# rdesc/autorally

Hardware: AMD Instinct MI355X
Metric: trajectory rollouts/s per MPPI solve (higher is better)
Workload: dtype f32

## Files before the change

### autorally_amd/csrc/group_roles.hpp

```cpp
#pragma once

#include "mppi_device.hpp"
#include "noise_device.hpp"

namespace mppi {

constexpr int kGRing = 16;
constexpr int kGCtlChunk = 4;

template <class SH>
struct GroupRoles {
  static constexpr int kPose = SH::NW, kCost = SH::NW + 1, kCtl = SH::NW + 2, kRng = SH::NW + 3;
  static constexpr int kWaves = SH::NW + 4;
  static_assert(kWaves <= (int)(sizeof(SH::fin) / sizeof(int)), "fin[]");
  static_assert(SH::kR == 16 || SH::kR == 8, "rollouts per group");
};
template <class SH>
__device__ __forceinline__ int group_j(int slot) { return slot & (SH::kR - 1); }
template <class SH>
__device__ __forceinline__ bool group_real(int slot) { return slot < SH::kR; }

template <class SH>
__device__ __forceinline__ int group_seq_min(SH &sh)
{
  int m = lds_peek(lds_addr(&sh.xseq[0][0]));
#pragma unroll
  for (int w = 1; w < SH::NW; w++) m = min(m, lds_peek(lds_addr(&sh.xseq[w][0])));
  return m;
}

struct MrgHalf {
  uint32_t s0, s1, s2;
};
__device__ __forceinline__ uint32_t fold_m(uint64_t x, uint32_t C, uint32_t m)
{
  x = (x >> 32) * C + (x & 0xffffffffULL);
  x = (x >> 32) * C + (x & 0xffffffffULL);
  x = (x >> 32) * C + (x & 0xffffffffULL);
  if (x >= m) x -= m;
  return (uint32_t)x;
}
template <class SH>
__device__ __forceinline__ MrgHalf group_rng_load(const RolloutArgs &a)
{
  const int lane = threadIdx.x & 63;
  const int j = group_j<SH>((lane >> 1) & 15), c = lane & 1;
  const int k = (int)blockIdx.x * SH::kR + j;
  const int K = a.K;
  MrgHalf g{0, 0, 0};
  if (a.inline_noise != 0 && lane < 2 * kRolloutsPerWave) {
    g.s0 = a.rng_in[(3 * c) * K + k]; g.s1 = a.rng_in[(3 * c + 1) * K + k]; g.s2 = a.rng_in[(3 * c + 2) * K + k];
  }
  return g;
}
template <class SH, bool PRE = false>
__device__ __forceinline__ void group_rng_wave(const RolloutArgs &a, SH &sh, const MrgHalf pre = MrgHalf{0, 0, 0})
{
  using R = GroupRoles<SH>;
  const int lane = threadIdx.x & 63;
  const int j = group_j<SH>((lane >> 1) & 15), c = lane & 1;
  const int k = (int)blockIdx.x * SH::kR + j;
  const int K = a.K, T = a.T;
  const bool active = lane < 2 * kRolloutsPerWave;
  const bool real = lane < 2 * SH::kR;
  int budget = spin_budget_init(a.spin_budget, T, a.fault_wave == R::kRng + 1);
  if (a.inline_noise != 0) {
    const uint32_t m = c ? (uint32_t)kM2 : (uint32_t)kM1, C = c ? kC2 : kC1;
    const uint32_t A = c ? (uint32_t)kA21 : (uint32_t)kA12, Bn = c ? (uint32_t)kA23N : (uint32_t)kA13N;
    MrgHalf g{0, 0, 0};
    if constexpr (PRE) {
      g = pre;
    } else if (active) {
      g.s0 = a.rng_in[(3 * c) * K + k]; g.s1 = a.rng_in[(3 * c + 1) * K + k]; g.s2 = a.rng_in[(3 * c + 2) * K + k];
    }
    const uint32_t a_ctl = lds_addr(&sh.ctl_pub[0]);
    const uint32_t a_mypub = lds_addr(&sh.rng_pub[lane]);
    int seen = 0;
    for (int t = 0; t < T; t++) {
      float2 e = make_float2(0.5f, 0.5f);
#ifdef MPPI_DIAG_NORNG
      e = make_float2(0.25f + 0.001f * (float)t, 0.5f);
#else
#pragma unroll
      for (int d = 0; d < 2; d++) {
        const uint32_t p = fold_m((uint64_t)A * (c ? g.s2 : g.s1) + (uint64_t)Bn * (m - g.s0), C, m);
        g.s0 = g.s1; g.s1 = g.s2; g.s2 = p;
        const uint32_t p2 = (uint32_t)__builtin_amdgcn_mov_dpp((int)p, 0xB1, 0xF, 0xF, false);
        uint32_t z = (p >= p2) ? p - p2 : p + (uint32_t)kM1 - p2;
        if (z == 0) z = (uint32_t)kM1;
        const float u = (float)z * 0x1p-32f;
        if (d == 0) e.x = u; else e.y = u;
      }
#endif
      const int need = t - kGRing + 1;
      while (seen < need && --budget > 0) {
        seen = lds_peek(a_ctl);
        if (seen < need) __builtin_amdgcn_s_sleep(2);
      }
      if (active && c == 0) *reinterpret_cast<float2 *>(&sh.eps[t & (kGRing - 1)][j][0]) = e;
      lds_publish(a_mypub, t + 1);
    }
    if (real) {
      a.rng_out[(3 * c) * K + k] = g.s0; a.rng_out[(3 * c + 1) * K + k] = g.s1; a.rng_out[(3 * c + 2) * K + k] = g.s2;
    }
  }
  spin_finish(budget, lds_addr(&sh.fail[0]), lds_addr(&sh.fin[R::kRng]));
}

template <class SH>
__device__ __forceinline__ void group_control_wave(const RolloutArgs &a, SH &sh, const uint32_t a_gate_open = 0)
{
  using R = GroupRoles<SH>;
  constexpr int NSW = SH::NSW;
  static_assert(kGCtlChunk == 4 && kGRing >= 2 * kGCtlChunk, "four steps per iteration, lanes 16 q + j");
  const int lane = threadIdx.x & 63;
  const int j = group_j<SH>(lane & 15), q = lane >> 4;
  const bool real = group_real<SH>(lane & 15);
  const int k = (int)blockIdx.x * SH::kR + j;
  const int K = a.K, T = a.T;
  const bool inl = a.inline_noise != 0;
  float2 *const noise = reinterpret_cast<float2 *>(a.noise);
  const float2 *const Useq = reinterpret_cast<const float2 *>(a.U);
  const bool noise_free_k = (k == 0);
  const bool pure_noise_k = (k >= a.k99);
  const uint32_t a_cd = lds_addr(&sh.cost_done[0]);
  const uint32_t a_mypub = lds_addr(&sh.ctl_pub[lane]);
  const uint32_t a_rng = lds_addr(&sh.rng_pub[0]);
  int budget = spin_budget_init(a.spin_budget, T, a.fault_wave == R::kCtl + 1);
  const bool gated = a_gate_open != 0;
  if (gated)
    while (lds_peek(a_gate_open) == 0 && --budget > 0) __builtin_amdgcn_s_sleep(1);
  int seen_x = 0, seen_c = 0, seen_r = 0;
  for (int t0 = 0, n = 1; t0 < T; t0 += n, n = kGCtlChunk) {
    const int t = t0 + q;
    const bool live = (t < T) & (q < n);
    const int tl = live ? t : T - 1;
    float2 Ut;
    if (gated) {
      const unsigned long long ub = __hip_atomic_load(reinterpret_cast<const unsigned long long *>(Useq + tl), __ATOMIC_RELAXED, __HIP_MEMORY_SCOPE_SYSTEM);
      Ut = make_float2(__uint_as_float((unsigned)ub), __uint_as_float((unsigned)(ub >> 32)));
    } else {
      Ut = Useq[tl];
    }
    float2 e = (live && !inl) ? noise[(size_t)tl * K + k] : make_float2(0.0f, 0.0f);
    const int tm = min(t0 + n, T) - 1;
    const int need_x = (tm >= kGRing) ? (tm - kGRing) * NSW + 1 : 0;
    const int need_c = tm - kGRing + 1;
    while ((seen_x < need_x || seen_c < need_c) && --budget > 0) {
      seen_x = group_seq_min(sh);
      seen_c = lds_peek(a_cd);
      if (seen_x < need_x || seen_c < need_c) __builtin_amdgcn_s_sleep(2);
    }
    if (inl) {
      while (seen_r < tm + 1 && --budget > 0) {
        seen_r = lds_peek(a_rng);
        if (seen_r < tm + 1) __builtin_amdgcn_s_sleep(1);
      }
#ifdef MPPI_DIAG_NOBM
      e = *reinterpret_cast<const float2 *>(&sh.eps[tl & (kGRing - 1)][j][0]);
#else
      e = box_muller(*reinterpret_cast<const float2 *>(&sh.eps[tl & (kGRing - 1)][j][0]));
#endif
    }
    if (live) {
      const bool nf = noise_free_k | (t < a.opt_delay);
      const float n0 = e.x * a.nu[0], n1 = e.y * a.nu[1];
      const float du0 = nf ? 0.0f : n0, du1 = nf ? 0.0f : n1;
      float u0 = nf ? Ut.x : (pure_noise_k ? n0 : Ut.x + n0);
      float u1 = nf ? Ut.y : (pure_noise_k ? n1 : Ut.y + n1);
      if (real) noise[(size_t)t * K + k] = make_float2(u0, u1);
      u0 = clampf(u0, a.u_lo[0], a.u_hi[0]);
      u1 = clampf(u1, a.u_lo[1], a.u_hi[1]);
      const int slot = t & (kGRing - 1);
      sh.ctl_b1[slot][j] = u0;
      sh.ctl_b1[slot][kRolloutsPerWave + j] = u1;
      *reinterpret_cast<float4 *>(&sh.ctl_rec[slot][j][0]) = make_float4(u0, u1, du0, du1);
    }
    lds_publish(a_mypub, tm + 1);
  }
  spin_finish(budget, lds_addr(&sh.fail[0]), lds_addr(&sh.fin[R::kCtl]));
}

template <class SH, bool AFFINE>
__device__ __forceinline__ void group_pose_wave(const RolloutArgs &a, SH &sh)
{
  using R = GroupRoles<SH>;
  constexpr int NSW = SH::NSW;
  static_assert(SH::kR == 16, "one step per iteration: 16-rollout groups only");
  const int lane = threadIdx.x & 63;
  const int j = lane & 15;
  const int T = a.T;
  const uint32_t a_seq0 = lds_addr(&sh.xseq[0][0]);
  const uint32_t a_cd = lds_addr(&sh.cost_done[0]);
  const uint32_t a_mypub = lds_addr(&sh.pose_pub[lane]);
  float x = a.state[0], y = a.state[1], yaw = a.state[2];
  int budget = spin_budget_init(a.spin_budget, T, a.fault_wave == R::kPose + 1), seen = 0, cdone = 0;
  float tf_p = 0.0f, tb_p = 0.0f;
  for (int t = 0; t <= T; t++) {
    float tf = 0.0f, tb = 0.0f;
    if (t < T) {
      const int need = t * NSW + 1;
      while (seen < need && --budget > 0) {
        seen = SH::kRecByAll ? group_seq_min(sh) : lds_peek(a_seq0);
        if (seen < need) __builtin_amdgcn_s_sleep(1);
      }
      const float4 r0 = *reinterpret_cast<const float4 *>(&sh.rec[t & (kGRing - 1)][j][0]);
      float spsi, cpsi;
#ifdef MPPI_DIAG_NOPOSE
      spsi = 0.0f; cpsi = 1.0f; tf = x; tb = y;
#else
      sincos_fast(yaw, spsi, cpsi);
      const float st[3] = {x, y, yaw};
      track_fetch<AFFINE>(a.cost, st, cpsi, spsi, tf, tb);
#endif
      const float sd0 = fmaf(cpsi, r0.y, -(spsi * r0.z));
      const float sd1 = fmaf(spsi, r0.y, cpsi * r0.z);
      const float sd2 = a.negate_yaw_der ? -r0.w : r0.w;
      x = fmaf(sd0, a.dt, x);
      y = fmaf(sd1, a.dt, y);
      yaw = fmaf(sd2, a.dt, yaw);
    }
    if (t > 0) {
      while (cdone < t - kGRing && --budget > 0) cdone = lds_peek(a_cd);
      if (lane < kRolloutsPerWave) *reinterpret_cast<float2 *>(&sh.tex[(t - 1) & (kGRing - 1)][lane][0]) = make_float2(tf_p, tb_p);
      lds_publish(a_mypub, t);
    }
    tf_p = tf; tb_p = tb;
  }
  spin_finish(budget, lds_addr(&sh.fail[0]), lds_addr(&sh.fin[R::kPose]));
}

template <int Q>
__device__ __forceinline__ float quad_bc(float v)
{
  return __int_as_float(__builtin_amdgcn_mov_dpp(__float_as_int(v), Q * 0x55, 0xF, 0xF, false));
}
__device__ __forceinline__ void quad_chain(float v, float d, float dt, int q, float &vq, float &v_out)
{
  const float v1 = fmaf(quad_bc<0>(d), dt, v);
  const float v2 = fmaf(quad_bc<1>(d), dt, v1);
  const float v3 = fmaf(quad_bc<2>(d), dt, v2);
  v_out = fmaf(quad_bc<3>(d), dt, v3);
  const float lo = (q == 0) ? v : v1, hi = (q == 2) ? v2 : v3;
  vq = (q < 2) ? lo : hi;
}
template <class SH, bool AFFINE>
__device__ __forceinline__ void group_pose_wave4(const RolloutArgs &a, SH &sh, const float x0, const float y0, const float yaw0,
                                                 const int budget_cut = 0);
template <class SH, bool AFFINE>
__device__ __forceinline__ void group_pose_wave4(const RolloutArgs &a, SH &sh)
{
  group_pose_wave4<SH, AFFINE>(a, sh, a.state[0], a.state[1], a.state[2]);
}
template <class SH, bool AFFINE>
__device__ __forceinline__ void group_pose_wave4(const RolloutArgs &a, SH &sh, const float x0, const float y0, const float yaw0,
                                                 const int budget_cut)
{
  using R = GroupRoles<SH>;
  constexpr int NSW = SH::NSW;
  static_assert(kRolloutsPerWave == 16 && kGRing >= 8, "lane = 4 j + q");
  const int lane = threadIdx.x & 63;
  const int j = group_j<SH>(lane >> 2), q = lane & 3;
  const int T = a.T;
  const uint32_t a_seq0 = lds_addr(&sh.xseq[0][0]);
  const uint32_t a_cd = lds_addr(&sh.cost_done[0]);
  const uint32_t a_mypub = lds_addr(&sh.pose_pub[lane]);
  float x = x0, y = y0, yaw = yaw0;
  int budget = spin_budget_init(a.spin_budget, T, a.fault_wave == R::kPose + 1 || budget_cut != 0), seen = 0, cdone = 0;
  for (int t0 = 0; t0 < T; t0 += 4) {
    const int t = t0 + q;
    const int tend = min(t0 + 4, T);
    const int need = (tend - 1) * NSW + 1;
    while (seen < need && --budget > 0) {
      seen = SH::kRecByAll ? group_seq_min(sh) : lds_peek(a_seq0);
      if (seen < need) __builtin_amdgcn_s_sleep(1);
    }
    const float4 r0 = *reinterpret_cast<const float4 *>(&sh.rec[t & (kGRing - 1)][j][0]);
    float yaw_q, yaw_n, x_q, x_n, y_q, y_n;
    quad_chain(yaw, a.negate_yaw_der ? -r0.w : r0.w, a.dt, q, yaw_q, yaw_n);
    float spsi, cpsi, tf = 0.0f, tb = 0.0f;
#ifdef MPPI_DIAG_NOPOSE
    spsi = 0.0f; cpsi = 1.0f;
#else
    sincos_fast(yaw_q, spsi, cpsi);
#endif
    quad_chain(x, fmaf(cpsi, r0.y, -(spsi * r0.z)), a.dt, q, x_q, x_n);
    quad_chain(y, fmaf(spsi, r0.y, cpsi * r0.z), a.dt, q, y_q, y_n);
#ifdef MPPI_DIAG_NOPOSE
    tf = x_q; tb = y_q;
#else
    const float st[3] = {x_q, y_q, yaw_q};
    track_fetch<AFFINE>(a.cost, st, cpsi, spsi, tf, tb);
#endif
    x = x_n; y = y_n; yaw = yaw_n;
    while (cdone < tend - kGRing && --budget > 0) cdone = lds_peek(a_cd);
    if (t < T) *reinterpret_cast<float2 *>(&sh.tex[t & (kGRing - 1)][j][0]) = make_float2(tf, tb);
    lds_publish(a_mypub, tend);
  }
  spin_finish(budget, lds_addr(&sh.fail[0]), lds_addr(&sh.fin[R::kPose]));
}

template <class SH>
__device__ __forceinline__ float group_settle(SH &sh, int budget, float J)
{
  using R = GroupRoles<SH>;
  const int lane = threadIdx.x & 63;
  const uint32_t a_fin = lds_addr(&sh.fin[(lane < R::kWaves) ? lane : 0]);
  for (;;) {
    const int v = (lane == R::kCost) ? 1 : lds_peek_lanes(a_fin);
    const bool all = __builtin_amdgcn_ballot_w64(v != 0) == ~0ull;
    if (all || --budget <= 0) break;
    __builtin_amdgcn_s_sleep(1);
  }
  if (budget <= 0 || lds_peek(lds_addr(&sh.fail[0])) != 0) J = __builtin_nanf("");
  return J;
}

template <class SH, bool CTRL>
__device__ __forceinline__ void group_cost_wave(const RolloutArgs &a, SH &sh)
{
  using R = GroupRoles<SH>;
  const int lane = threadIdx.x & 63;
  static_assert(SH::kR == 16, "one step per iteration: 16-rollout groups only");
  const int j = lane & 15;
  const int k = (int)blockIdx.x * kRolloutsPerWave + j;
  const int T = a.T;
  const uint32_t a_mydone = lds_addr(&sh.cost_done[lane]);
  const uint32_t a_pose = lds_addr(&sh.pose_pub[0]);
  int crash = 0, budget = spin_budget_init(a.spin_budget, T, a.fault_wave == R::kCost + 1), seen = 0;
  float J = 0.0f;
  for (int t = 0; t < T; t++) {
    const double rt = a.inv_t[t];
    while (seen < t + 1 && --budget > 0) {
      seen = lds_peek(a_pose);
      if (seen < t + 1) __builtin_amdgcn_s_sleep(1);
    }
    const float4 r0 = *reinterpret_cast<const float4 *>(&sh.rec[t & (kGRing - 1)][j][0]);
    const float4 r1 = *reinterpret_cast<const float4 *>(&sh.ctl_rec[t & (kGRing - 1)][j][0]);
    const float2 tx = *reinterpret_cast<const float2 *>(&sh.tex[t & (kGRing - 1)][j][0]);
    lds_publish(a_mydone, t + 1);
    const int rc = (int)((t > 0) & (fabsf(r0.x) >= kRollCrash));
#ifdef MPPI_DIAG_NOCOST
    crash |= rc;
    int crash_new = crash;
    const float Jn = J + r0.y + r1.x + tx.x + (float)rt;
#else
    CostTerms ct;
    cost_terms_a<CTRL>(a.cost, a.nu, r0.y, r0.z, r1.x, r1.y, r1.z, r1.w, ct);
    crash |= rc;
    int crash_new = crash;
    const float c = cost_terms_b(a.cost, ct, tx.x, tx.y, crash_new);
    const float Jn = running_mean(J, c, t, rt);
#endif
    J = (t > 0) ? Jn : J;
    crash = (t > 0) ? crash_new : crash;
  }
  J = group_settle(sh, budget, J);
  a.costs[k] = J + 0.0f;
}

template <int Q>
__device__ __forceinline__ int quad_bc_i(int v)
{
  return __builtin_amdgcn_mov_dpp(v, Q * 0x55, 0xF, 0xF, false);
}
template <class SH, bool CTRL>
__device__ __forceinline__ void group_cost_wave4(const RolloutArgs &a, SH &sh)
{
  using R = GroupRoles<SH>;
  const int lane = threadIdx.x & 63;
  const int j = group_j<SH>(lane >> 2), q = lane & 3;
  const int k = (int)blockIdx.x * SH::kR + j;
  const int T = a.T;
  const uint32_t a_mydone = lds_addr(&sh.cost_done[lane]);
  const uint32_t a_pose = lds_addr(&sh.pose_pub[0]);
  int crash = 0, budget = spin_budget_init(a.spin_budget, T, a.fault_wave == R::kCost + 1), seen = 0;
  float J = 0.0f;
  for (int t0 = 0; t0 < T; t0 += 4) {
    const int t = t0 + q;
    const int tend = min(t0 + 4, T);
    while (seen < tend && --budget > 0) {
      seen = lds_peek(a_pose);
      if (seen < tend) __builtin_amdgcn_s_sleep(1);
    }
    const float4 r0 = *reinterpret_cast<const float4 *>(&sh.rec[t & (kGRing - 1)][j][0]);
    const float4 r1 = *reinterpret_cast<const float4 *>(&sh.ctl_rec[t & (kGRing - 1)][j][0]);
    const float2 tx = *reinterpret_cast<const float2 *>(&sh.tex[t & (kGRing - 1)][j][0]);
    lds_publish(a_mydone, tend);
    const bool counted = (t > 0) & (t < T);
    int e = (int)(fabsf(r0.x) >= kRollCrash) | (int)(tx.x >= a.cost.boundary_threshold) | (int)(tx.y >= a.cost.boundary_threshold);
    e = counted ? e : 0;
    const int c0 = crash | quad_bc_i<0>(e), c1 = c0 | quad_bc_i<1>(e), c2 = c1 | quad_bc_i<2>(e), c3 = c2 | quad_bc_i<3>(e);
    const int lo = (q == 0) ? c0 : c1, hi = (q == 2) ? c2 : c3;
    int crash_q = (q < 2) ? lo : hi;
    crash = c3;
#ifdef MPPI_DIAG_NOCOST
    const float c = r0.y + r1.x + tx.x + (float)crash_q;
#else
    CostTerms ct;
    cost_terms_a<CTRL>(a.cost, a.nu, r0.y, r0.z, r1.x, r1.y, r1.z, r1.w, ct);
    const float c = cost_terms_b(a.cost, ct, tx.x, tx.y, crash_q);
#endif
#pragma unroll
    for (int l = 0; l < 4; l++) {
      const int tl = t0 + l;
      const float cl = (l == 0) ? quad_bc<0>(c) : (l == 1) ? quad_bc<1>(c) : (l == 2) ? quad_bc<2>(c) : quad_bc<3>(c);
      if (tl > 0 && tl < T) {
#ifdef MPPI_DIAG_NOCOST
        J = J + cl + (float)a.inv_t[tl];
#else
        J = running_mean(J, cl, tl, a.inv_t[tl]);
#endif
      }
    }
  }
  J = group_settle(sh, budget, J);
  if (q == 0 && group_real<SH>(lane >> 2)) a.costs[k] = J + 0.0f;
}

}
```

### autorally_amd/csrc/rollout_row.hip

```cpp
#include "group_roles.hpp"
#include "mppi_kernels.hpp"

namespace mppi {

#ifdef MPPI_ROW_STAMPS
__device__ unsigned long long g_row_stamps[16];
#define RSTAMP(i)                                                                                         \
  do {                                                                                                    \
    if (blockIdx.x == 0 && (threadIdx.x & 63) == 0) {                                                     \
      unsigned long long t__;                                                                             \
      asm volatile("s_memtime %0\n\ts_waitcnt lgkmcnt(0)" : "=s"(t__)::"memory");                           \
      g_row_stamps[i] = t__;                                                                              \
    }                                                                                                     \
  } while (0)
#else
#define RSTAMP(i) do { } while (0)
#endif

template <int H>
struct RowShared {
  static constexpr int NW = 4;
  static constexpr int NSW = 1;
  static constexpr bool kRecByAll = true;
  static constexpr int kR = 16;
  int xseq[NW][64];
  float rec[kGRing][kRolloutsPerWave][4];
  int cost_done[64];
  float ctl_b1[kGRing][64];
  float ctl_rec[kGRing][kRolloutsPerWave][4];
  int ctl_pub[64];
  float tex[kGRing][kRolloutsPerWave][2];
  int pose_pub[64];
  float eps[kGRing][kRolloutsPerWave][2];
  int rng_pub[64];
  int fail[4];
  int fin[8];
  float gstate[8];
  int gate_open[8];
  float dump[NW][64 * 2 + (kGRing - 1) * kRolloutsPerWave * 4];
};

template <int H, bool TREE>
struct RowWeights {
  f32x2 w1[kNetIn], w2[H], w3[TREE ? 4 : H];
  f32x2 b1s, b2s, b3;
};

constexpr int kRowPackEntries = 40;
template <int H, bool TREE>
__device__ __forceinline__ void row_load(const float *rowpack, int p, RowWeights<H, TREE> &W)
{
  static_assert(H == 32, "entry layout of pack_row_weights");
  const float4 *pk = reinterpret_cast<const float4 *>(rowpack) + p;
#pragma unroll
  for (int i = 0; i < 3; i++) {
    const float4 v = pk[i * 16];
    W.w1[2 * i] = f32x2{v.x, v.y};
    W.w1[2 * i + 1] = f32x2{v.z, v.w};
  }
#pragma unroll
  for (int i = 0; i < H / 2; i++) {
    const float4 v = pk[(3 + i) * 16];
    W.w2[2 * i] = f32x2{v.x, v.y};
    W.w2[2 * i + 1] = f32x2{v.z, v.w};
    if constexpr (!TREE) {
      const float4 u = pk[(3 + H / 2 + i) * 16];
      W.w3[2 * i] = f32x2{u.x, u.y};
      W.w3[2 * i + 1] = f32x2{u.z, u.w};
    }
  }
  const float4 b = pk[35 * 16];
  W.b1s = f32x2{b.x, b.y};
  W.b2s = f32x2{b.z, b.w};
  if constexpr (TREE) {
    const float4 u = pk[37 * 16], v = pk[38 * 16], c = pk[39 * 16];
    W.w3[0] = f32x2{u.x, u.y};
    W.w3[1] = f32x2{u.z, u.w};
    W.w3[2] = f32x2{v.x, v.y};
    W.w3[3] = f32x2{v.z, v.w};
    W.b3 = f32x2{c.x, c.y};
  } else {
    const float4 c = pk[36 * 16];
    W.b3 = f32x2{c.x, c.y};
  }
}

template <int Q>
__device__ __forceinline__ float row_bc(float a)
{
  return __int_as_float(__builtin_amdgcn_mov_dpp(__float_as_int(a), 0x150 + Q, 0xF, 0xF, false));
}
template <int Q>
__device__ __forceinline__ f32x2 row_bc2(f32x2 a)
{
  return __builtin_bit_cast(f32x2, (long long)__builtin_amdgcn_mov_dpp(__builtin_bit_cast(long long, a), 0x150 + Q, 0xF, 0xF, false));
}
template <int Q>
__device__ __forceinline__ void row_dot_step(f32x2 &z, f32x2 &b, const f32x2 *w, f32x2 a)
{
  z = __builtin_elementwise_fma(w[2 * Q], f32x2{b.x, b.x}, z);
  __builtin_amdgcn_sched_barrier(0);
  const f32x2 bn = row_bc2<(Q + 1 < 16 ? Q + 1 : 15)>(a);
  __builtin_amdgcn_sched_barrier(0);
  z = __builtin_elementwise_fma(w[2 * Q + 1], f32x2{b.y, b.y}, z);
  __builtin_amdgcn_sched_barrier(0);
  b = bn;
}
__device__ __forceinline__ f32x2 row_dot_bc(const f32x2 *w, f32x2 a)
{
  f32x2 z = {0.0f, 0.0f};
  f32x2 b = row_bc2<0>(a);
  __builtin_amdgcn_sched_barrier(0);
#define RD4(Q) row_dot_step<Q>(z, b, w, a); row_dot_step<Q + 1>(z, b, w, a); row_dot_step<Q + 2>(z, b, w, a); row_dot_step<Q + 3>(z, b, w, a);
  RD4(0) RD4(4) RD4(8) RD4(12)
#undef RD4
  return z;
}

template <int CTRL>
__device__ __forceinline__ float dpp_add(float acc, float src)
{
  return acc + __int_as_float(__builtin_amdgcn_update_dpp(0, __float_as_int(src), CTRL, 0xF, 0xF, true));
}
__device__ __forceinline__ float row_out_tree(const f32x2 *w3, f32x2 a)
{
  const f32x2 ax = {a.x, a.x}, ay = {a.y, a.y};
  const f32x2 v01 = __builtin_elementwise_fma(w3[1], ay, w3[0] * ax);
  const f32x2 v23 = __builtin_elementwise_fma(w3[3], ay, w3[2] * ax);
  float v0 = dpp_add<0x128>(v01.x, v23.x);
  const float v1 = dpp_add<0x128>(v01.y, v23.y);
  v0 = dpp_add<0x141>(v0, v1);
  v0 = dpp_add<0xB1>(v0, v0);
  v0 = dpp_add<0x4E>(v0, v0);
  return v0;
}

template <int H, bool TREE, bool GATED = false>
__device__ __forceinline__ void row_dynamics(const RolloutArgs &a, RowShared<H> &sh, const int w)
{
  static_assert(H == 32, "row_dot_bc: 32 activations, two per lane of a 16-lane row");
  const int lane = threadIdx.x & 63;
  const int r = lane >> 4, p = lane & 15;
  const int jr = 4 * w + r;
  const bool odd = (p & 1) != 0;
  const int T = a.T;
  RowWeights<H, TREE> W;
  row_load<H, TREE>(a.wpack, p, W);
#pragma unroll
  for (int k = 0; k < H; k++) asm volatile("" : "+v"(W.w2[k]));
#pragma unroll
  for (int k = 0; k < (TREE ? 4 : H); k++) asm volatile("" : "+v"(W.w3[k]));

  const uint32_t a_myseq = lds_addr(&sh.xseq[w][lane]);
  typedef const volatile int __attribute__((address_space(3))) *lds_int_p;
  typedef const volatile f32x2 __attribute__((address_space(3))) *lds_f2_p;
  const lds_int_p p_pub = (lds_int_p)&sh.ctl_pub[0];
  const lds_f2_p p_u = (lds_f2_p)&sh.ctl_rec[0][jr][0];
  constexpr int kSlotF2 = kRolloutsPerWave * 2;
  const uint32_t a_rec0 = TREE ? (((p & 3) == 0) ? lds_addr(&sh.rec[0][jr][p >> 2]) : lds_addr(&sh.dump[w][2 * lane]))
                               : ((p < 2) ? lds_addr(&sh.rec[0][jr][2 * p]) : lds_addr(&sh.dump[w][2 * lane]));
  constexpr uint32_t kRecStride = sizeof(float) * kRolloutsPerWave * 4;

  int budget = spin_budget_init(a.spin_budget, T, a.fault_wave == w + 1);
  f32x2 sp;
  if constexpr (GATED) {
    const uint32_t a_go = lds_addr(&sh.gate_open[0]);
    while (lds_peek(a_go) == 0 && --budget > 0) __builtin_amdgcn_s_sleep(1);
    const volatile float *gs = sh.gstate;
    sp = TREE ? f32x2{gs[3 + (p >> 2)], 0.0f} : odd ? f32x2{gs[5], gs[6]} : f32x2{gs[3], gs[4]};
  } else {
    sp = TREE ? f32x2{a.state[3 + (p >> 2)], 0.0f} : odd ? f32x2{a.state[5], a.state[6]} : f32x2{a.state[3], a.state[4]};
  }
  if (w == 0) RSTAMP(2);
  while (__builtin_amdgcn_readfirstlane(*p_pub) < 1 && --budget > 0) __builtin_amdgcn_s_sleep(1);
  if (w == 0) RSTAMP(3);
  f32x2 un = p_u[0];
  asm volatile("" : "+v"(un));

  for (int t = 0; t < T - 1; t++) {
    const int slot = t & (kGRing - 1);
    const f32x2 u = un;
    const f32x2 slo = TREE ? f32x2{row_bc<0>(sp.x), row_bc<4>(sp.x)} : f32x2{row_bc<0>(sp.x), row_bc<0>(sp.y)};
    const f32x2 shi = TREE ? f32x2{row_bc<8>(sp.x), row_bc<12>(sp.x)} : f32x2{row_bc<1>(sp.x), row_bc<1>(sp.y)};
    if constexpr (TREE) asm volatile("ds_write_b32 %0, %1" ::"v"(a_rec0 + (uint32_t)slot * kRecStride), "v"(sp.x) : "memory");
    else asm volatile("ds_write_b64 %0, %1" ::"v"(a_rec0 + (uint32_t)slot * kRecStride), "v"(sp) : "memory");
    lds_publish(a_myseq, t + 1);
    f32x2 z = {0.0f, 0.0f};
    z = __builtin_elementwise_fma(W.w1[0], f32x2{slo.x, slo.x}, z);
    z = __builtin_elementwise_fma(W.w1[1], f32x2{slo.y, slo.y}, z);
    z = __builtin_elementwise_fma(W.w1[2], f32x2{shi.x, shi.x}, z);
    z = __builtin_elementwise_fma(W.w1[3], f32x2{shi.y, shi.y}, z);
    z = __builtin_elementwise_fma(W.w1[4], f32x2{u.x, u.x}, z);
    z = __builtin_elementwise_fma(W.w1[5], f32x2{u.y, u.y}, z);
    const int sn = ((t + 1) & (kGRing - 1)) * kSlotF2;
    const int cp_v = *p_pub;
    un = p_u[sn];
    const f32x2 a0 = tanh_bias2(z, W.b1s);
    const f32x2 a1 = tanh_bias2(row_dot_bc(W.w2, a0), W.b2s);
    const int want = t + 2;
    const int cp_e = __builtin_amdgcn_readfirstlane(cp_v);
    asm volatile("" : "+v"(un));
    if constexpr (TREE) {
      const float d = row_out_tree(W.w3, a1) + W.b3.x;
      sp.x = fmaf(d, a.dt, sp.x);
      asm volatile("" : "+v"(sp.x));
    } else {
      const f32x2 d = row_dot_bc(W.w3, a1) + W.b3;
      sp = __builtin_elementwise_fma(d, f32x2{a.dt, a.dt}, sp);
      asm volatile("" : "+v"(sp));
    }
    if (__builtin_expect(cp_e < want, 0)) {
      int cp = cp_e;
      while (cp < want && --budget > 0) {
        cp = __builtin_amdgcn_readfirstlane(*p_pub);
        un = p_u[sn];
      }
      asm volatile("" : "+v"(un));
    }
  }
  if (w == 0) RSTAMP(4);
  {
    const int t = T - 1;
    if constexpr (TREE) asm volatile("ds_write_b32 %0, %1" ::"v"(a_rec0 + (uint32_t)(t & (kGRing - 1)) * kRecStride), "v"(sp.x) : "memory");
    else asm volatile("ds_write_b64 %0, %1" ::"v"(a_rec0 + (uint32_t)(t & (kGRing - 1)) * kRecStride), "v"(sp) : "memory");
    lds_publish(a_myseq, t + 1);
  }
  spin_finish(budget, lds_addr(&sh.fail[0]), lds_addr(&sh.fin[w]));
}

template <int H, bool AFFINE, bool CTRL, bool TREE, bool GATED = false>
__device__ __forceinline__ void row_group(const RolloutArgs &a, RowShared<H> &sh)
{
  using SH = RowShared<H>;
  using R = GroupRoles<SH>;
  const int lane = threadIdx.x & 63;
  const int role = __builtin_amdgcn_readfirstlane(threadIdx.x >> 6);
  if (role == 0) RSTAMP(0);
  MrgHalf g0{0, 0, 0};
  if (role == R::kRng) g0 = group_rng_load<SH>(a);
  if (role == 0) {
#pragma unroll
    for (int w = 0; w < 4; w++) sh.xseq[w][lane] = 0;
    sh.cost_done[lane] = 0;
    sh.ctl_pub[lane] = 0;
    sh.pose_pub[lane] = 0;
    sh.rng_pub[lane] = 0;
    sh.fail[lane & 3] = 0;
    sh.fin[lane & 7] = 0;
    sh.gate_open[lane & 7] = 0;
  }
  __syncthreads();
  if (role == 0) RSTAMP(1);
#ifdef MPPI_ROW_RIDER_PRIO
  if (role >= 4) __builtin_amdgcn_s_setprio(MPPI_ROW_RIDER_PRIO);
#endif
  if (role < 4) row_dynamics<H, TREE, GATED>(a, sh, role);
  else if (role == R::kCost) { group_cost_wave4<SH, CTRL>(a, sh); RSTAMP(5); }
  else if (role == R::kCtl) { group_control_wave(a, sh, GATED ? lds_addr(&sh.gate_open[0]) : 0u); RSTAMP(6); }
  else if (role == R::kPose) {
    if constexpr (GATED) {
      const int shut = group_gate_wait(a, sh);
      const volatile float *gs = sh.gstate;
      const float x0 = gs[0], y0 = gs[1], yaw0 = gs[2];
      group_pose_wave4<SH, AFFINE>(a, sh, x0, y0, yaw0, shut);
    } else {
      group_pose_wave4<SH, AFFINE>(a, sh);
    }
    RSTAMP(7);
  }
  else { group_rng_wave<SH, true>(a, sh, g0); RSTAMP(8); }
}

template <int H, bool AFFINE, bool CTRL, bool TREE>
__global__ __launch_bounds__(512) void rollout_row_kernel(const RolloutArgs a)
{
  __shared__ __attribute__((aligned(16))) RowShared<H> sh;
  row_group<H, AFFINE, CTRL, TREE>(a, sh);
}
template <int H, bool AFFINE, bool CTRL, bool TREE>
__global__ __launch_bounds__(512) void rollout_row_gated_kernel(const RolloutArgs a)
{
  __shared__ __attribute__((aligned(16))) RowShared<H> sh;
  row_group<H, AFFINE, CTRL, TREE, true>(a, sh);
}

template <int H, bool AFFINE, bool CTRL, bool TREE, int NB>
__global__ __launch_bounds__(512) void rollout_row_batch_kernel(const QuadBatchArgsT<NB> b)
{
  __shared__ __attribute__((aligned(16))) RowShared<H> sh;
#define MPPI_ROW_BODY(A)                                                                                   \
  do {                                                                                                     \
    if ((int)blockIdx.x >= (A).K / kRolloutsPerWave) return;      \
    row_group<H, AFFINE, CTRL, TREE>((A), sh);                                                             \
  } while (0)
  MPPI_BATCH_DISPATCH(NB, b, MPPI_ROW_BODY);
#undef MPPI_ROW_BODY
}

template <int H, bool AFFINE, bool CTRL, bool TREE, int NB>
__global__ __launch_bounds__(512) void rollout_row_batch_gated_kernel(const QuadBatchArgsT<NB> b)
{
  __shared__ __attribute__((aligned(16))) RowShared<H> sh;
#define MPPI_ROW_BODY(A)                                                                                   \
  do {                                                                                                     \
    if ((int)blockIdx.x >= (A).K / kRolloutsPerWave) return;      \
    row_group<H, AFFINE, CTRL, TREE, true>((A), sh);                                                       \
  } while (0)
  MPPI_BATCH_DISPATCH(NB, b, MPPI_ROW_BODY);
#undef MPPI_ROW_BODY
}

bool row_variant_supported(int hidden, int n_hidden) { return hidden == 32 && n_hidden == 2; }
int row_pack_floats() { return kRowPackEntries * 16 * 4; }

#define MPPI_ROW_DISPATCH(LAUNCH, KERN, TREE, ...)                                                            \
  do {                                                                                                        \
    if (affine && !ctrl) LAUNCH((KERN<32, true, false, TREE>), __VA_ARGS__);                                  \
    else if (affine && ctrl) LAUNCH((KERN<32, true, true, TREE>), __VA_ARGS__);                               \
    else if (!affine && !ctrl) LAUNCH((KERN<32, false, false, TREE>), __VA_ARGS__);                           \
    else LAUNCH((KERN<32, false, true, TREE>), __VA_ARGS__);                                                  \
  } while (0)
#define MPPI_ROW_BATCH_DISPATCH(KERN, TREE, NB, ...)                                                                            \
  do {                                                                                                                          \
    if (affine && !ctrl) hipLaunchKernelGGL((KERN<32, true, false, TREE, NB>), __VA_ARGS__);                                    \
    else if (affine && ctrl) hipLaunchKernelGGL((KERN<32, true, true, TREE, NB>), __VA_ARGS__);                                 \
    else if (!affine && !ctrl) hipLaunchKernelGGL((KERN<32, false, false, TREE, NB>), __VA_ARGS__);                             \
    else hipLaunchKernelGGL((KERN<32, false, true, TREE, NB>), __VA_ARGS__);                                                    \
  } while (0)

hipError_t launch_rollout_row_batch(const QuadBatchArgs &b, bool tree, hipStream_t stream)
{
  if (b.n < 1 || b.n > kMaxBatch) return hipErrorInvalidValue;
  bool affine = true, ctrl = false;
  int gmax = 0;
  const bool gated = b.inst[0].gate != nullptr;
  for (int i = 0; i < b.n; i++) {
    if ((b.inst[i].gate != nullptr) != gated) return hipErrorInvalidValue;
    affine = affine && b.inst[i].cost.affine != 0;
    ctrl = ctrl || b.inst[i].cost.need_control_cost != 0;
    gmax = b.inst[i].K / kRolloutsPerWave > gmax ? b.inst[i].K / kRolloutsPerWave : gmax;
  }
  const dim3 grid(gmax, b.n), block(512);
  if (b.n <= 2) {
    const QuadBatchArgsT<2> b2 = batch_args_prefix<2>(b);
    if (gated) {
      if (tree) MPPI_ROW_BATCH_DISPATCH(rollout_row_batch_gated_kernel, true, 2, grid, block, 0, stream, b2);
      else MPPI_ROW_BATCH_DISPATCH(rollout_row_batch_gated_kernel, false, 2, grid, block, 0, stream, b2);
    } else {
      if (tree) MPPI_ROW_BATCH_DISPATCH(rollout_row_batch_kernel, true, 2, grid, block, 0, stream, b2);
      else MPPI_ROW_BATCH_DISPATCH(rollout_row_batch_kernel, false, 2, grid, block, 0, stream, b2);
    }
  } else {
    if (gated) {
      if (tree) MPPI_ROW_BATCH_DISPATCH(rollout_row_batch_gated_kernel, true, 4, grid, block, 0, stream, b);
      else MPPI_ROW_BATCH_DISPATCH(rollout_row_batch_gated_kernel, false, 4, grid, block, 0, stream, b);
    } else {
      if (tree) MPPI_ROW_BATCH_DISPATCH(rollout_row_batch_kernel, true, 4, grid, block, 0, stream, b);
      else MPPI_ROW_BATCH_DISPATCH(rollout_row_batch_kernel, false, 4, grid, block, 0, stream, b);
    }
  }
  return hipGetLastError();
}

hipError_t launch_rollout_row(int hidden, int n_hidden, const RolloutArgs &a, bool tree, hipStream_t stream)
{
  if (!row_variant_supported(hidden, n_hidden) || a.K % kRolloutsPerWave != 0) return hipErrorInvalidValue;
  const bool affine = a.cost.affine != 0, ctrl = a.cost.need_control_cost != 0;
  const dim3 grid(a.K / kRolloutsPerWave), block(512);
  if (a.gate != nullptr) {
    if (tree) MPPI_ROW_DISPATCH(MPPI_LAUNCH_ROLLOUT, rollout_row_gated_kernel, true, grid, block, 0, stream, a);
    else MPPI_ROW_DISPATCH(MPPI_LAUNCH_ROLLOUT, rollout_row_gated_kernel, false, grid, block, 0, stream, a);
    return hipGetLastError();
  }
  if (tree) MPPI_ROW_DISPATCH(MPPI_LAUNCH_ROLLOUT, rollout_row_kernel, true, grid, block, 0, stream, a);
  else MPPI_ROW_DISPATCH(MPPI_LAUNCH_ROLLOUT, rollout_row_kernel, false, grid, block, 0, stream, a);
  return hipGetLastError();
}
#undef MPPI_ROW_DISPATCH
#undef MPPI_ROW_BATCH_DISPATCH

}

#ifdef MPPI_ROW_STAMPS
extern "C" int mppi_debug_read_row_stamps(unsigned long long *out)
{
  return (int)hipMemcpyFromSymbol(out, HIP_SYMBOL(mppi::g_row_stamps), sizeof(unsigned long long) * 16);
}
#endif
```

Baseline: 102.7 million.

## Loosen pose and cost wave waits on dynamics records to overlap more work

The pose wave now waits only for records up to the third step of each 4-step block. It computes sincos, the integration and the track fetch for those steps, then waits for the last step's record to finish propagating the carried state. The cost wave waits on the dynamics sequence instead of pose publication before loading records, computing the control/speed cost terms and prefetching inv_t, and only then waits for pose output. This aims to shorten the critical path across the producer-consumer waves, at the cost of extra spin-wait loops and LDS reads. The debug stamp array also grows to record hardware IDs per wave.

```diff
diff --git a/autorally_amd/csrc/group_roles.hpp b/autorally_amd/csrc/group_roles.hpp
--- a/autorally_amd/csrc/group_roles.hpp
+++ b/autorally_amd/csrc/group_roles.hpp
@@ -235,15 +235,15 @@
 {
   return __int_as_float(__builtin_amdgcn_mov_dpp(__float_as_int(v), Q * 0x55, 0xF, 0xF, false));
 }
-__device__ __forceinline__ void quad_chain(float v, float d, float dt, int q, float &vq, float &v_out)
+__device__ __forceinline__ void quad_chain3(float v, float d, float dt, int q, float &vq, float &v3)
 {
   const float v1 = fmaf(quad_bc<0>(d), dt, v);
   const float v2 = fmaf(quad_bc<1>(d), dt, v1);
-  const float v3 = fmaf(quad_bc<2>(d), dt, v2);
-  v_out = fmaf(quad_bc<3>(d), dt, v3);
+  v3 = fmaf(quad_bc<2>(d), dt, v2);
   const float lo = (q == 0) ? v : v1, hi = (q == 2) ? v2 : v3;
   vq = (q < 2) ? lo : hi;
 }
+__device__ __forceinline__ float quad_last(float v3, float d, float dt) { return fmaf(quad_bc<3>(d), dt, v3); }
 template <class SH, bool AFFINE>
 __device__ __forceinline__ void group_pose_wave4(const RolloutArgs &a, SH &sh, const float x0, const float y0, const float yaw0,
                                                  const int budget_cut = 0);
@@ -270,29 +270,39 @@
   for (int t0 = 0; t0 < T; t0 += 4) {
     const int t = t0 + q;
     const int tend = min(t0 + 4, T);
-    const int need = (tend - 1) * NSW + 1;
+    const int need = (tend - 2) * NSW + 1;
     while (seen < need && --budget > 0) {
       seen = SH::kRecByAll ? group_seq_min(sh) : lds_peek(a_seq0);
       if (seen < need) __builtin_amdgcn_s_sleep(1);
     }
-    const float4 r0 = *reinterpret_cast<const float4 *>(&sh.rec[t & (kGRing - 1)][j][0]);
-    float yaw_q, yaw_n, x_q, x_n, y_q, y_n;
-    quad_chain(yaw, a.negate_yaw_der ? -r0.w : r0.w, a.dt, q, yaw_q, yaw_n);
+    float4 r0 = *reinterpret_cast<const float4 *>(&sh.rec[t & (kGRing - 1)][j][0]);
+    float yaw_q, yaw_3, x_q, x_3, y_q, y_3;
+    quad_chain3(yaw, a.negate_yaw_der ? -r0.w : r0.w, a.dt, q, yaw_q, yaw_3);
     float spsi, cpsi, tf = 0.0f, tb = 0.0f;
 #ifdef MPPI_DIAG_NOPOSE
     spsi = 0.0f; cpsi = 1.0f;
 #else
     sincos_fast(yaw_q, spsi, cpsi);
 #endif
-    quad_chain(x, fmaf(cpsi, r0.y, -(spsi * r0.z)), a.dt, q, x_q, x_n);
-    quad_chain(y, fmaf(spsi, r0.y, cpsi * r0.z), a.dt, q, y_q, y_n);
+    quad_chain3(x, fmaf(cpsi, r0.y, -(spsi * r0.z)), a.dt, q, x_q, x_3);
+    quad_chain3(y, fmaf(spsi, r0.y, cpsi * r0.z), a.dt, q, y_q, y_3);
 #ifdef MPPI_DIAG_NOPOSE
     tf = x_q; tb = y_q;
 #else
     const float st[3] = {x_q, y_q, yaw_q};
     track_fetch<AFFINE>(a.cost, st, cpsi, spsi, tf, tb);
 #endif
-    x = x_n; y = y_n; yaw = yaw_n;
+    if (tend < T) {
+      const int need3 = (tend - 1) * NSW + 1;
+      while (seen < need3 && --budget > 0) {
+        seen = SH::kRecByAll ? group_seq_min(sh) : lds_peek(a_seq0);
+        if (seen < need3) __builtin_amdgcn_s_sleep(1);
+      }
+      r0 = *reinterpret_cast<const float4 *>(&sh.rec[t & (kGRing - 1)][j][0]);
+      yaw = quad_last(yaw_3, a.negate_yaw_der ? -r0.w : r0.w, a.dt);
+      x = quad_last(x_3, fmaf(cpsi, r0.y, -(spsi * r0.z)), a.dt);
+      y = quad_last(y_3, fmaf(spsi, r0.y, cpsi * r0.z), a.dt);
+    }
     while (cdone < tend - kGRing && --budget > 0) cdone = lds_peek(a_cd);
     if (t < T) *reinterpret_cast<float2 *>(&sh.tex[t & (kGRing - 1)][j][0]) = make_float2(tf, tb);
     lds_publish(a_mypub, tend);
@@ -374,21 +384,36 @@
   const int T = a.T;
   const uint32_t a_mydone = lds_addr(&sh.cost_done[lane]);
   const uint32_t a_pose = lds_addr(&sh.pose_pub[0]);
-  int crash = 0, budget = spin_budget_init(a.spin_budget, T, a.fault_wave == R::kCost + 1), seen = 0;
+  const uint32_t a_seq0 = lds_addr(&sh.xseq[0][0]);
+  int crash = 0, budget = spin_budget_init(a.spin_budget, T, a.fault_wave == R::kCost + 1), seen = 0, seen_r = 0;
   float J = 0.0f;
   for (int t0 = 0; t0 < T; t0 += 4) {
     const int t = t0 + q;
     const int tend = min(t0 + 4, T);
+    const int need_r = (tend - 1) * SH::NSW + 1;
+    while (seen_r < need_r && --budget > 0) {
+      seen_r = SH::kRecByAll ? group_seq_min(sh) : lds_peek(a_seq0);
+      if (seen_r < need_r) __builtin_amdgcn_s_sleep(1);
+    }
+    const float4 r0 = *reinterpret_cast<const float4 *>(&sh.rec[t & (kGRing - 1)][j][0]);
+    const float4 r1 = *reinterpret_cast<const float4 *>(&sh.ctl_rec[t & (kGRing - 1)][j][0]);
+    const bool counted = (t > 0) & (t < T);
+    const int e_roll = (int)(fabsf(r0.x) >= kRollCrash);
+    double rt[4];
+#pragma unroll
+    for (int l = 0; l < 4; l++) rt[l] = a.inv_t[min(max(t0 + l, 1), T - 1)];
+#ifndef MPPI_DIAG_NOCOST
+    CostTerms ct;
+    cost_terms_a<CTRL>(a.cost, a.nu, r0.y, r0.z, r1.x, r1.y, r1.z, r1.w, ct);
+    asm volatile("" : "+v"(ct.control_cost), "+v"(ct.speed_cost), "+v"(ct.stabilizing_cost));
+#endif
     while (seen < tend && --budget > 0) {
       seen = lds_peek(a_pose);
       if (seen < tend) __builtin_amdgcn_s_sleep(1);
     }
-    const float4 r0 = *reinterpret_cast<const float4 *>(&sh.rec[t & (kGRing - 1)][j][0]);
-    const float4 r1 = *reinterpret_cast<const float4 *>(&sh.ctl_rec[t & (kGRing - 1)][j][0]);
     const float2 tx = *reinterpret_cast<const float2 *>(&sh.tex[t & (kGRing - 1)][j][0]);
     lds_publish(a_mydone, tend);
-    const bool counted = (t > 0) & (t < T);
-    int e = (int)(fabsf(r0.x) >= kRollCrash) | (int)(tx.x >= a.cost.boundary_threshold) | (int)(tx.y >= a.cost.boundary_threshold);
+    int e = e_roll | (int)(tx.x >= a.cost.boundary_threshold) | (int)(tx.y >= a.cost.boundary_threshold);
     e = counted ? e : 0;
     const int c0 = crash | quad_bc_i<0>(e), c1 = c0 | quad_bc_i<1>(e), c2 = c1 | quad_bc_i<2>(e), c3 = c2 | quad_bc_i<3>(e);
     const int lo = (q == 0) ? c0 : c1, hi = (q == 2) ? c2 : c3;
@@ -397,8 +422,6 @@
 #ifdef MPPI_DIAG_NOCOST
     const float c = r0.y + r1.x + tx.x + (float)crash_q;
 #else
-    CostTerms ct;
-    cost_terms_a<CTRL>(a.cost, a.nu, r0.y, r0.z, r1.x, r1.y, r1.z, r1.w, ct);
     const float c = cost_terms_b(a.cost, ct, tx.x, tx.y, crash_q);
 #endif
 #pragma unroll
@@ -407,9 +430,9 @@
       const float cl = (l == 0) ? quad_bc<0>(c) : (l == 1) ? quad_bc<1>(c) : (l == 2) ? quad_bc<2>(c) : quad_bc<3>(c);
       if (tl > 0 && tl < T) {
 #ifdef MPPI_DIAG_NOCOST
-        J = J + cl + (float)a.inv_t[tl];
-#else
-        J = running_mean(J, cl, tl, a.inv_t[tl]);
+        J = J + cl + (float)rt[l];
+#else
+        J = running_mean(J, cl, tl, rt[l]);
 #endif
       }
     }
diff --git a/autorally_amd/csrc/rollout_row.hip b/autorally_amd/csrc/rollout_row.hip
--- a/autorally_amd/csrc/rollout_row.hip
+++ b/autorally_amd/csrc/rollout_row.hip
@@ -4,7 +4,7 @@
 namespace mppi {
 
 #ifdef MPPI_ROW_STAMPS
-__device__ unsigned long long g_row_stamps[16];
+__device__ unsigned long long g_row_stamps[32];
 #define RSTAMP(i)                                                                                         \
   do {                                                                                                    \
     if (blockIdx.x == 0 && (threadIdx.x & 63) == 0) {                                                     \
@@ -251,6 +251,13 @@
   }
   __syncthreads();
   if (role == 0) RSTAMP(1);
+#ifdef MPPI_ROW_STAMPS
+  if (blockIdx.x == 0 && lane == 0) {
+    unsigned hw;
+    asm volatile("s_getreg_b32 %0, hwreg(HW_REG_HW_ID)" : "=s"(hw));
+    g_row_stamps[16 + role] = hw;
+  }
+#endif
 #ifdef MPPI_ROW_RIDER_PRIO
   if (role >= 4) __builtin_amdgcn_s_setprio(MPPI_ROW_RIDER_PRIO);
 #endif
@@ -384,6 +391,6 @@
 #ifdef MPPI_ROW_STAMPS
 extern "C" int mppi_debug_read_row_stamps(unsigned long long *out)
 {
-  return (int)hipMemcpyFromSymbol(out, HIP_SYMBOL(mppi::g_row_stamps), sizeof(unsigned long long) * 16);
+  return (int)hipMemcpyFromSymbol(out, HIP_SYMBOL(mppi::g_row_stamps), sizeof(unsigned long long) * 32);
 }
 #endif
```

Result: faster. 104.6 million, median of 6 (+1.9%).

## Unroll row dynamics by four steps and batch progress publishing and polling

Applied to the files above, without the earlier changes.

Splits the per-timestep body of the row dynamics into a templated step that is unrolled four times per chunk. Within a chunk the ring slot offsets become compile-time immediates on the LDS writes and control reads. The progress counter is published only on the fourth step, and the control-publisher counter is read only on the first step of each chunk. This cuts address arithmetic and LDS synchronisation traffic on the serial critical path. In exchange, consumers of the published sequence see progress in coarser four-step jumps, which could delay downstream roles. It also relies on a stale counter value for three of the four steps, which may trigger more frequent spin waits.

```diff
diff --git a/autorally_amd/csrc/rollout_row.hip b/autorally_amd/csrc/rollout_row.hip
--- a/autorally_amd/csrc/rollout_row.hip
+++ b/autorally_amd/csrc/rollout_row.hip
@@ -135,10 +135,61 @@
   return v0;
 }
 
+template <int H, bool TREE, int Q>
+__device__ __forceinline__ void row_step(const RolloutArgs &a, const RowWeights<H, TREE> &W, f32x2 &sp, f32x2 &un, const int t0,
+                                         const uint32_t a_rec, const uint32_t a_myseq, const volatile int __attribute__((address_space(3))) *p_pub,
+                                         const volatile f32x2 __attribute__((address_space(3))) *&pu,
+                                         const volatile f32x2 __attribute__((address_space(3))) *p_u0, int &cp, int &budget)
+{
+  constexpr int kSlotF2 = kRolloutsPerWave * 2;
+  constexpr uint32_t kRecStride = sizeof(float) * kRolloutsPerWave * 4;
+  const int t = t0 + Q;
+  const f32x2 u = un;
+  const f32x2 slo = TREE ? f32x2{row_bc<0>(sp.x), row_bc<4>(sp.x)} : f32x2{row_bc<0>(sp.x), row_bc<0>(sp.y)};
+  const f32x2 shi = TREE ? f32x2{row_bc<8>(sp.x), row_bc<12>(sp.x)} : f32x2{row_bc<1>(sp.x), row_bc<1>(sp.y)};
+  if constexpr (TREE) asm volatile("ds_write_b32 %0, %1 offset:%2" ::"v"(a_rec), "v"(sp.x), "n"(Q * kRecStride) : "memory");
+  else asm volatile("ds_write_b64 %0, %1 offset:%2" ::"v"(a_rec), "v"(sp), "n"(Q * kRecStride) : "memory");
+  if constexpr (Q == 3) lds_publish(a_myseq, t + 1);
+  f32x2 z = {0.0f, 0.0f};
+  z = __builtin_elementwise_fma(W.w1[0], f32x2{slo.x, slo.x}, z);
+  z = __builtin_elementwise_fma(W.w1[1], f32x2{slo.y, slo.y}, z);
+  z = __builtin_elementwise_fma(W.w1[2], f32x2{shi.x, shi.x}, z);
+  z = __builtin_elementwise_fma(W.w1[3], f32x2{shi.y, shi.y}, z);
+  z = __builtin_elementwise_fma(W.w1[4], f32x2{u.x, u.x}, z);
+  z = __builtin_elementwise_fma(W.w1[5], f32x2{u.y, u.y}, z);
+  int cp_v = 0;
+  if constexpr (Q == 0) cp_v = *p_pub;
+  if constexpr (Q == 3) pu = p_u0 + ((t + 1) & (kGRing - 1)) * kSlotF2;
+  constexpr int kUn = (Q == 3) ? 0 : (Q + 1) * kSlotF2;
+  un = pu[kUn];
+  const f32x2 a0 = tanh_bias2(z, W.b1s);
+  const f32x2 a1 = tanh_bias2(row_dot_bc(W.w2, a0), W.b2s);
+  const int want = t + 2;
+  if constexpr (Q == 0) cp = __builtin_amdgcn_readfirstlane(cp_v);
+  asm volatile("" : "+v"(un));
+  if constexpr (TREE) {
+    const float d = row_out_tree(W.w3, a1) + W.b3.x;
+    sp.x = fmaf(d, a.dt, sp.x);
+    asm volatile("" : "+v"(sp.x));
+  } else {
+    const f32x2 d = row_dot_bc(W.w3, a1) + W.b3;
+    sp = __builtin_elementwise_fma(d, f32x2{a.dt, a.dt}, sp);
+    asm volatile("" : "+v"(sp));
+  }
+  if (__builtin_expect(cp < want, 0)) {
+    while (cp < want && --budget > 0) {
+      cp = __builtin_amdgcn_readfirstlane(*p_pub);
+      un = pu[kUn];
+    }
+    asm volatile("" : "+v"(un));
+  }
+}
+
 template <int H, bool TREE, bool GATED = false>
 __device__ __forceinline__ void row_dynamics(const RolloutArgs &a, RowShared<H> &sh, const int w)
 {
   static_assert(H == 32, "row_dot_bc: 32 activations, two per lane of a 16-lane row");
+  static_assert(kGRing % 4 == 0, "aligned chunks of four steps inside the ring");
   const int lane = threadIdx.x & 63;
   const int r = lane >> 4, p = lane & 15;
   const int jr = 4 * w + r;
@@ -155,8 +206,9 @@
   typedef const volatile int __attribute__((address_space(3))) *lds_int_p;
   typedef const volatile f32x2 __attribute__((address_space(3))) *lds_f2_p;
   const lds_int_p p_pub = (lds_int_p)&sh.ctl_pub[0];
-  const lds_f2_p p_u = (lds_f2_p)&sh.ctl_rec[0][jr][0];
-  constexpr int kSlotF2 = kRolloutsPerWave * 2;
+  uint32_t a_u0 = lds_addr(&sh.ctl_rec[0][jr][0]);
+  asm volatile("" : "+v"(a_u0));
+  const lds_f2_p p_u = (lds_f2_p)a_u0;
   const uint32_t a_rec0 = TREE ? (((p & 3) == 0) ? lds_addr(&sh.rec[0][jr][p >> 2]) : lds_addr(&sh.dump[w][2 * lane]))
                                : ((p < 2) ? lds_addr(&sh.rec[0][jr][2 * p]) : lds_addr(&sh.dump[w][2 * lane]));
   constexpr uint32_t kRecStride = sizeof(float) * kRolloutsPerWave * 4;
@@ -172,51 +224,23 @@
     sp = TREE ? f32x2{a.state[3 + (p >> 2)], 0.0f} : odd ? f32x2{a.state[5], a.state[6]} : f32x2{a.state[3], a.state[4]};
   }
   if (w == 0) RSTAMP(2);
-  while (__builtin_amdgcn_readfirstlane(*p_pub) < 1 && --budget > 0) __builtin_amdgcn_s_sleep(1);
+  int cp = 0;
+  while ((cp = __builtin_amdgcn_readfirstlane(*p_pub)) < 1 && --budget > 0) __builtin_amdgcn_s_sleep(1);
   if (w == 0) RSTAMP(3);
-  f32x2 un = p_u[0];
+  lds_f2_p pu = p_u;
+  f32x2 un = pu[0];
   asm volatile("" : "+v"(un));
 
-  for (int t = 0; t < T - 1; t++) {
-    const int slot = t & (kGRing - 1);
-    const f32x2 u = un;
-    const f32x2 slo = TREE ? f32x2{row_bc<0>(sp.x), row_bc<4>(sp.x)} : f32x2{row_bc<0>(sp.x), row_bc<0>(sp.y)};
-    const f32x2 shi = TREE ? f32x2{row_bc<8>(sp.x), row_bc<12>(sp.x)} : f32x2{row_bc<1>(sp.x), row_bc<1>(sp.y)};
-    if constexpr (TREE) asm volatile("ds_write_b32 %0, %1" ::"v"(a_rec0 + (uint32_t)slot * kRecStride), "v"(sp.x) : "memory");
-    else asm volatile("ds_write_b64 %0, %1" ::"v"(a_rec0 + (uint32_t)slot * kRecStride), "v"(sp) : "memory");
-    lds_publish(a_myseq, t + 1);
-    f32x2 z = {0.0f, 0.0f};
-    z = __builtin_elementwise_fma(W.w1[0], f32x2{slo.x, slo.x}, z);
-    z = __builtin_elementwise_fma(W.w1[1], f32x2{slo.y, slo.y}, z);
-    z = __builtin_elementwise_fma(W.w1[2], f32x2{shi.x, shi.x}, z);
-    z = __builtin_elementwise_fma(W.w1[3], f32x2{shi.y, shi.y}, z);
-    z = __builtin_elementwise_fma(W.w1[4], f32x2{u.x, u.x}, z);
-    z = __builtin_elementwise_fma(W.w1[5], f32x2{u.y, u.y}, z);
-    const int sn = ((t + 1) & (kGRing - 1)) * kSlotF2;
-    const int cp_v = *p_pub;
-    un = p_u[sn];
-    const f32x2 a0 = tanh_bias2(z, W.b1s);
-    const f32x2 a1 = tanh_bias2(row_dot_bc(W.w2, a0), W.b2s);
-    const int want = t + 2;
-    const int cp_e = __builtin_amdgcn_readfirstlane(cp_v);
-    asm volatile("" : "+v"(un));
-    if constexpr (TREE) {
-      const float d = row_out_tree(W.w3, a1) + W.b3.x;
-      sp.x = fmaf(d, a.dt, sp.x);
-      asm volatile("" : "+v"(sp.x));
-    } else {
-      const f32x2 d = row_dot_bc(W.w3, a1) + W.b3;
-      sp = __builtin_elementwise_fma(d, f32x2{a.dt, a.dt}, sp);
-      asm volatile("" : "+v"(sp));
-    }
-    if (__builtin_expect(cp_e < want, 0)) {
-      int cp = cp_e;
-      while (cp < want && --budget > 0) {
-        cp = __builtin_amdgcn_readfirstlane(*p_pub);
-        un = p_u[sn];
-      }
-      asm volatile("" : "+v"(un));
-    }
+  const int NS = T - 1;
+  for (int t0 = 0; t0 < NS; t0 += 4) {
+    const uint32_t a_rec = a_rec0 + (uint32_t)(t0 & (kGRing - 1)) * kRecStride;
+    row_step<H, TREE, 0>(a, W, sp, un, t0, a_rec, a_myseq, p_pub, pu, p_u, cp, budget);
+    if (t0 + 1 >= NS) break;
+    row_step<H, TREE, 1>(a, W, sp, un, t0, a_rec, a_myseq, p_pub, pu, p_u, cp, budget);
+    if (t0 + 2 >= NS) break;
+    row_step<H, TREE, 2>(a, W, sp, un, t0, a_rec, a_myseq, p_pub, pu, p_u, cp, budget);
+    if (t0 + 3 >= NS) break;
+    row_step<H, TREE, 3>(a, W, sp, un, t0, a_rec, a_myseq, p_pub, pu, p_u, cp, budget);
   }
   if (w == 0) RSTAMP(4);
   {
```

New measurement: 102.3 million before, 106.4 million after, median of 6. 4.0% higher.
